# bernborgess/raft-tla

Measured on AMD Instinct MI355X. Metric: distinct states/sec (whole node) + wall time to exhaust, 3-server Raft, higher is better.
Workload: dtype u32

## Files before the change

### raft-tla_amd/csrc/rtla_klevel.h

```cpp
#pragma once
#include "rtla_kdev.h"

namespace {

template <int NS>
__device__ __forceinline__ void add_at(uint32_t* a, uint32_t j, uint32_t v) {
#pragma unroll
  for (int k = 0; k < NS; k++)
    if ((uint32_t)k == j) a[k] += v;
}
template <int NS, int S, class P>
__device__ __forceinline__ int successor_orbit_step_sig(const Layout& L, P prow, const DeltaT<NS>& d,
                                                        const uint32_t* psg, int k, bool all, FP& best) {
  return with_successor<NS>(L, prow, d, [&](auto rec_of, int nmsg, auto slot_of, int nelec, auto elec_of) {
    uint32_t ms[NS], mr[NS];
#pragma unroll
    for (int j = 0; j < NS; j++) {
      ms[j] = psg[(NS + j) * S];
      mr[j] = psg[(2 * NS + j) * S];
    }
#pragma unroll
    for (int q = 0; q < 3; q++) {
      if (q >= d.nops) continue;
      const uint64_t o = d.op_old[q], v = d.op_new[q];
      if (o) {
        const uint32_t c = slot_sig_sent(L, o);
        add_at<NS>(ms, slot_src(L, o), 0u - c);
        add_at<NS>(mr, slot_dst(L, o), 0u - slot_sig_recv(c));
      }
      if (v) {
        const uint32_t c = slot_sig_sent(L, v);
        add_at<NS>(ms, slot_src(L, v), c);
        add_at<NS>(mr, slot_dst(L, v), slot_sig_recv(c));
      }
    }
    const uint32_t lsrv = d.srv >= 0 ? srv_sig<NS>(d.srv, d.rec) : 0u;
    uint64_t sig[NS];
#pragma unroll
    for (int i = 0; i < NS; i++) sig[i] = sig_of(i == d.srv ? lsrv : psg[i * S], ms[i], mr[i]);
    const SymRank r = sym_rank_from<NS>(L, sig, rec_of, nmsg, slot_of, nelec, elec_of);
    const int k1 = all ? r.ncomb : min(k + 1, r.ncomb);
    for (int j = k; j < k1; j++) {
      const FP f = sym_image_fp<NS>(L, rec_of, nmsg, slot_of, nelec, elec_of, r, j);
      if (fp_less(f, best)) best = f;
    }
    return k1 < r.ncomb ? k1 : -1;
  });
}

}

namespace {

constexpr int RING = 128;
constexpr int NEWCAP = 512;
constexpr int NEWFLUSH = NEWCAP - 3 * 64;


__host__ __device__ constexpr int compact_lds_words(int W, int AW, int GROUP, bool sym, bool multi) {
  return (4 * GROUP * (sym ? 2 : 1) + (multi ? 4 * SHARD_MAX : 0) + NEWCAP / 2 + GROUP * W + GROUP * AW +
          RING / 2 * (sym ? 2 : 1) + (sym ? 5 * 64 + 3 * NMAX * GROUP : 0) + 3) & ~3;
}

__device__ __forceinline__ unsigned long long win_bits(unsigned long long bits, int off) {
  if (off >= 64 || off <= -64) return 0ull;
  return off >= 0 ? bits << off : bits >> (-off);
}

template <int NS>
__device__ __forceinline__ unsigned long long cand_mask(const Layout& L, const uint32_t* row, int nmsg, int wb,
                                                        bool dup = true) {
  constexpr int N = NS;
  unsigned long long rv = 0, bl = 0, ldr = 0, tmo = 0;
#pragma unroll
  for (int i = 0; i < N; i++) {
    const uint32_t w0 = srv_w0(L, row, i);
    const uint32_t role = s_role(w0);
    if (role == FOLLOWER || role == CANDIDATE) tmo |= 1ull << i;
    if (role == CANDIDATE) {
      rv |= (unsigned long long)(~s_vresp(w0) & ((1u << N) - 1u)) << (i * N);
      if (__builtin_popcount(s_vgrant(w0)) * 2 > N) bl |= 1ull << i;
    }
    if (role == LEADER) ldr |= 1ull << i;
  }
  unsigned long long ae = 0, cr = 0;
#pragma unroll
  for (int i = 0; i < N; i++)
    if (ldr >> i & 1ull) {
      ae |= (((1ull << N) - 1ull) & ~(1ull << i)) << (i * N);
      cr |= ((1ull << L.V) - 1ull) << (i * L.V);
    }
  const unsigned long long bag = nmsg >= 64 ? ~0ull : ((1ull << nmsg) - 1ull);
  unsigned long long m = 0;
  m |= win_bits((1ull << N) - 1ull, L.fam[F_RESTART] - wb);
  m |= win_bits(tmo, L.fam[F_TIMEOUT] - wb);
  m |= win_bits(rv, L.fam[F_REQUESTVOTE] - wb);
  m |= win_bits(bl, L.fam[F_BECOMELEADER] - wb);
  m |= win_bits(cr, L.fam[F_CLIENTREQUEST] - wb);
  m |= win_bits(ldr, L.fam[F_ADVANCECOMMIT] - wb);
  m |= win_bits(ae, L.fam[F_APPENDENTRIES] - wb);
  m |= win_bits(bag, L.fam[F_RECEIVE] - wb);
  if (dup) m |= win_bits(bag, L.fam[F_DUPLICATE] - wb);
  m |= win_bits(bag, L.fam[F_DROP] - wb);
  return m;
}

__device__ __forceinline__ void outbox_holes(const ShardBox& box, int o, unsigned long long from,
                                             unsigned long long to, int lane) {
  to = min(to, box.cap);
  for (unsigned long long j = from + lane; j < to; j += 64) {
    const unsigned long long k = (unsigned long long)o * box.cap + j;
    box.send_fp[2 * k] = 0ull;
    box.send_fp[2 * k + 1] = 0ull;
  }
}

__device__ __forceinline__ unsigned long long home_slot(const FP& key, int lg) {
  return lg ? key.a >> (64 - lg) : 0ull;
}

}

#ifndef RTLA_COMPACT_WAVES_PER_EU
#define RTLA_COMPACT_WAVES_PER_EU 3
#endif
#ifndef RTLA_SYM_WAVES_PER_EU
#define RTLA_SYM_WAVES_PER_EU 4
#endif

namespace {
struct KeyStep {
  FP f;
  int next;
};
template <int NS, Layout LC, int S>
__device__ __noinline__ KeyStep key_one(const Layout& Lrt, const uint32_t* prow, const uint32_t* psg, int inst, int k,
                                        bool all, FP best0, FP afp) {
  const Layout& L = pick_layout<LC>(Lrt);
  DeltaT<NS> d;
  d.enabled = 0;
  compute_delta<NS>(L, prow, inst, d);
  KeyStep r{FP{0, 0}, -1};
  if (!d.enabled) {
    r.next = -2;
    return r;
  }
  FP best = best0;
  r.next = successor_orbit_step_sig<NS, S>(L, prow, d, psg, k, all, best);
  r.f = r.next < 0 ? fp_add(orbit_key_finish(best), afp) : best;
  return r;
}

struct BuildOut {
  int bad, sub, in_model;
};
template <int NS, Layout LC, int GROUP>
__device__ __noinline__ BuildOut build_one(const Layout& Lrt, const uint32_t* prow, int inst, FP qfp,
                                           const uint32_t* pall_p, uint32_t* d1, uint32_t* base2, int n1, int off,
                                           bool write, bool wait) {
  const Layout& L = pick_layout<LC>(Lrt);
  DeltaT<NS> d;
  d.enabled = 0;
  compute_delta<NS>(L, prow, inst, d);
  const FP cfp = fp_add(qfp, delta_fp<NS>(L, prow, d));
  BuildOut o{check_invariants_v<NS>(L, prow, d.srv, d.rec[0], d.rec[1], d.elec, d.erec[0]), d.sub, d.in_model};
  uint32_t spk[PACKW], epk[PACKW];
  child_pack(L, d, spk, epk);
  if (wait) asm volatile("s_waitcnt vmcnt(0)" ::: "memory");
  if (write)
    child_write(L, prow, d, spk, epk, StridedWords<GROUP>{const_cast<uint32_t*>(pall_p)}, cfp, [&](int w, uint32_t v) {
      const int i = off + w;
      if (i < n1) d1[i] = v;
      else base2[i - n1] = v;
    });
  return o;
}

}

#ifdef RTLA_STAMPS
#define RTLA_STAMP_DECL                                                   \
  unsigned long long st_prev_ = __builtin_amdgcn_s_memtime();              \
  unsigned long long st_acc_[8] = {0, 0, 0, 0, 0, 0, 0, 0};
#define STAMP(k)                                                             \
  do {                                                                       \
    const unsigned long long t_ = __builtin_amdgcn_s_memtime();              \
    st_acc_[k] += t_ - st_prev_;                                             \
    st_prev_ = t_;                                                           \
  } while (0)
#define RTLA_STAMP_FLUSH(ctr, lane)                                          \
  if ((lane) == 0)                                                           \
    for (int k_ = 0; k_ < 8; k_++) atomicAdd(&(ctr)->stamp[k_], st_acc_[k_]);
#else
#define RTLA_STAMP_DECL
#define STAMP(k)
#define RTLA_STAMP_FLUSH(ctr, lane)
#endif

#ifndef RTLA_NARROW_W
#define RTLA_NARROW_W 32
#endif
#ifndef RTLA_NARROW_WAVES
#define RTLA_NARROW_WAVES 4
#endif
constexpr int compact_waves(const Layout& L, bool sym) {
  return sym ? RTLA_SYM_WAVES_PER_EU
             : (L.N != 0 && L.W <= RTLA_NARROW_W ? RTLA_NARROW_WAVES : RTLA_COMPACT_WAVES_PER_EU);
}
template <int NS, bool MULTI, int GROUP, Layout LC, bool SYM>
__global__ void __launch_bounds__(256)
__attribute__((amdgpu_waves_per_eu(compact_waves(LC, SYM))))
k_expand_compact(Layout Lrt, Ring cur, unsigned long long s_begin, unsigned long long s_end,
                 unsigned long long cur_base, Ring next, unsigned long long* __restrict__ parents,
                 unsigned long long next_base, unsigned long long next_cap, unsigned long long* table,
                 unsigned long long* sent, int tlog2, DevCounters* ctr, ShardBox box, int xflags) {
  const Layout& L = pick_layout<LC>(Lrt);
  const int me = box.me;
  extern __shared__ __attribute__((aligned(16))) uint32_t lds[];
  __shared__ unsigned int cov[2 * COVER_CODES];
  const int wave = threadIdx.x >> 6, lane = threadIdx.x & 63;
  const int W = L.W, AW = L.all_words;
  uint32_t* wl = lds + wave * compact_lds_words(W, AW, GROUP, SYM, MULTI);
  FP* pfpl = reinterpret_cast<FP*>(wl);
  FP* afpl = pfpl + GROUP;
  unsigned long long* obox =
      reinterpret_cast<unsigned long long*>(wl + 4 * GROUP * (SYM ? 2 : 1));
  uint16_t* newl = reinterpret_cast<uint16_t*>(obox + (MULTI ? 2 * SHARD_MAX : 0));
  uint32_t* rows = reinterpret_cast<uint32_t*>(newl + NEWCAP);
  uint32_t* pall = rows + GROUP * W;
  const StridedWords<GROUP> pall_mine{pall + (lane & (GROUP - 1))};
  uint16_t* ring = reinterpret_cast<uint16_t*>(pall + GROUP * AW);
  uint16_t* kring = ring + RING;
  int kpos = 0, kdone = 0;
  FP* cbest = reinterpret_cast<FP*>(kring + (SYM ? RING : 0));
  uint32_t* cent = reinterpret_cast<uint32_t*>(cbest + (SYM ? 64 : 0));
  int ccount = 0;
  uint32_t* sigl = cent + (SYM ? 64 : 0);
  if (MULTI) {
    if (lane < SHARD_MAX) {
      obox[lane] = ~0ull;
      obox[SHARD_MAX + lane] = OBOX_CHUNK;
    }
    wave_sync();
  }
  cover_zero(cov, 2 * COVER_CODES);

  unsigned my_gen = 0, my_probe = 0;
  unsigned my_dup = 0;
#ifdef RTLA_COUNT_CAS
  unsigned my_cas = 0;
#endif
  const int ninst = L.fam[F_COUNT];
  const unsigned long long lanes_below = (1ull << lane) - 1ull;
  constexpr bool narrow = !SYM && LC.N != 0 && LC.W <= RTLA_NARROW_W;
  constexpr bool dup_narrow = false;
  const bool dup_counted = (!narrow || dup_narrow) && L.C == 1 && !(xflags & (XF_ALL_SUCCESSORS | XF_NO_CHUNKS));
  const bool recv_group = SYM || L.C > 1;
  constexpr int family_cut = narrow ? 22 : SYM ? 40 : 64;
  RTLA_STAMP_DECL
  bool pend = false;
  unsigned long long pold = 0;
  FP pf{0, 0};
  uint32_t pinfo = 0;
  const bool async_cas = !(xflags & XF_CAS_ONLY);
  bool cpend = false;
  bool cflight = false;
  unsigned long long cold = 0, ckey = 0, cidx = 0;
  uint32_t cinfo = 0;
  int head = 0, tail = 0;
  unsigned long long dedup_new = 0;
  unsigned long long s0 = 0;

  auto chunk_delta = [&](bool active, const uint32_t* prow, int inst, auto& d) {
    const int f0 = inst_family(L, __builtin_amdgcn_readfirstlane(inst));
    const bool one_family = __ballot(active && inst_family(L, inst) != f0) == 0ull;
    if (!one_family || (xflags & XF_GENERIC_DELTA)) {
      if (active) compute_delta<NS>(L, prow, inst, d);
    } else if (active) {
      switch (f0) {
        case F_RESTART: compute_delta<NS, F_RESTART>(L, prow, inst, d); break;
        case F_TIMEOUT: compute_delta<NS, F_TIMEOUT>(L, prow, inst, d); break;
        case F_REQUESTVOTE: compute_delta<NS, F_REQUESTVOTE>(L, prow, inst, d); break;
        case F_BECOMELEADER: compute_delta<NS, F_BECOMELEADER>(L, prow, inst, d); break;
        case F_CLIENTREQUEST: compute_delta<NS, F_CLIENTREQUEST>(L, prow, inst, d); break;
        case F_ADVANCECOMMIT: compute_delta<NS, F_ADVANCECOMMIT>(L, prow, inst, d); break;
        case F_APPENDENTRIES: compute_delta<NS, F_APPENDENTRIES>(L, prow, inst, d); break;
        case F_RECEIVE: compute_delta<NS, F_RECEIVE>(L, prow, inst, d); break;
        case F_DUPLICATE: compute_delta<NS, F_DUPLICATE>(L, prow, inst, d); break;
        default: compute_delta<NS, F_DROP>(L, prow, inst, d); break;
      }
    }
  };
  auto cover_add = [&](unsigned* base, bool on, int inst, int sub) {
    if (xflags & XF_NO_COVER) return;
    const int code = on ? cover_code(L, inst, sub) : -1;
    const unsigned long long m = __ballot(on);
    if (m) {
      const int c0 = __shfl(code, __builtin_ctzll(m));
      const bool same = on && code == c0;
      const int n0 = __popcll(__ballot(same));
      if (lane == 0) atomicAdd(&base[c0], (unsigned)n0);
      if (on && !same) atomicAdd(&base[code], 1u);
    }
  };
  auto build_all = [&]() {
    const int ntot = tail - head;
    if (ntot == 0) return;
    unsigned long long obase = 0;
    if (lane == 0) obase = atomicAdd(&ctr->next_count, (unsigned long long)ntot);
    obase = shfl0_u64(obase);
    if (obase + ntot > next_cap && lane == 0) set_flag(ctr, FLAG_FRONTIER_FULL);
    const int nrows = obase >= next_cap ? 0 : (int)min<unsigned long long>((unsigned long long)ntot, next_cap - obase);
    const bool rows_on = !(xflags & XF_NO_MATERIALIZE) && RTLA_IDX_OK(ctr, obase + nrows, ctr->cap_next + 1);
    const unsigned long long p0 = ring_idx(next, obase);
    const int n1 = (int)min<unsigned long long>(next.cap - p0, (unsigned long long)nrows) * W;
    uint32_t* d1 = next.base + p0 * (unsigned long long)W;
    auto copy_rows = [&](int rb, int re) {
      const int nwords = re * W;
      int r = rb, w = lane;
      while (w >= W) { w -= W; r++; }
      for (int i0 = rb * W; i0 < nwords; i0 += 64) {
        const int i = i0 + lane;
        if (i < nwords) {
          const int sr = newl[(head + r) & (NEWCAP - 1)] >> 8;
          const uint32_t v = rows[sr * W + w];
          if (i < n1) d1[i] = v;
          else next.base[i - n1] = v;
        }
        w += 64;
        while (w >= W) { w -= W; r++; }
      }
    };
    if (rows_on) copy_rows(0, nrows);
    for (int b = 0; b < ntot; b += 64) {
      const bool act = b + lane < ntot;
      const int e = act ? newl[(head + b + lane) & (NEWCAP - 1)] : 0;
      const int sl = e >> 8, inst = e & 255;
      const int child = b + lane;
      if constexpr (SYM) {
        BuildOut o{0, 0, 0};
        if (act)
          o = build_one<NS, LC, GROUP>(Lrt, rows + sl * W, inst, pfpl[sl], pall + sl, d1, next.base, n1, child * W,
                                      rows_on && child < nrows, rows_on && b == 0);
        else if (rows_on && b == 0)
          asm volatile("s_waitcnt vmcnt(0)" ::: "memory");
        if (!(xflags & XF_ALL_SUCCESSORS) && claim_violation(ctr, o.bad, lane))
          record_violation(ctr, cur_base + s0 + sl, inst, 1, child < nrows ? next_base + obase + child : ~0ull);
        cover_add(cov + COVER_CODES, act, inst, o.sub);
        if (child < nrows && RTLA_IDX_OK(ctr, next_base + obase + child, ctr->cap_parents))
          parents[next_base + obase + child] =
              (xflags & XF_ALL_SUCCESSORS)
                  ? (cur_base + s0 + sl) << 32 | (unsigned long long)(o.in_model ? 1u : 0u) << 31 |
                        (unsigned long long)o.sub << 16 | (unsigned long long)inst
                  : (unsigned long long)me << 56 | (cur_base + s0 + sl) << 16 | (unsigned long long)inst;
        continue;
      }
      DeltaT<NS> d;
      d.enabled = 0;
      if (act) compute_delta<NS>(L, rows + sl * W, inst, d);
      const FP qfp = pfpl[sl];
      FP cfp{0, 0};
      int bad = 0;
      if (act) {
        const uint32_t* prow = rows + sl * W;
        cfp = fp_add(qfp, delta_fp<NS>(L, prow, d));
        bad = check_invariants_v<NS>(L, prow, d.srv, d.rec[0], d.rec[1], d.elec, d.erec[0]);
      }
      if (!(xflags & XF_ALL_SUCCESSORS) && claim_violation(ctr, bad, lane))
        record_violation(ctr, cur_base + s0 + sl, inst, 1, child < nrows ? next_base + obase + child : ~0ull);
      cover_add(cov + COVER_CODES, act, inst, d.sub);
      uint32_t spk[PACKW], epk[PACKW];
      if (act) child_pack(L, d, spk, epk);
      if (rows_on) {
        if (b == 0) asm volatile("s_waitcnt vmcnt(0)" ::: "memory");
        if (child < nrows) {
          const StridedWords<GROUP> pall_p{pall + sl};
          const int off = child * W;
          child_write(L, rows + sl * W, d, spk, epk, pall_p, cfp, [&](int w, uint32_t v) {
            const int i = off + w;
            if (i < n1) d1[i] = v;
            else next.base[i - n1] = v;
          });
        }
      }
      if (child < nrows && RTLA_IDX_OK(ctr, next_base + obase + child, ctr->cap_parents))
        parents[next_base + obase + child] =
            (xflags & XF_ALL_SUCCESSORS)
                ? (cur_base + s0 + sl) << 32 | (unsigned long long)(d.in_model ? 1u : 0u) << 31 |
                      (unsigned long long)d.sub << 16 | (unsigned long long)inst
                : (unsigned long long)me << 56 | (cur_base + s0 + sl) << 16 | (unsigned long long)inst;
    }
    head = tail;
  };
  auto issue_cas = [&]() {
#ifdef RTLA_COUNT_CAS
    if (cpend) my_cas++;
#endif
    if (cpend) cold = atomicCAS(&table[cidx], 0ull, ckey);
    cflight = cpend;
    cpend = false;
  };
  auto resolve = [&]() {
    bool isnew = false;
    uint32_t ninfo = pinfo;
    const int powner = MULTI ? fp_owner(pf, box.nshard) : me;
    bool rem = false;
    if (xflags & XF_ALL_SUCCESSORS) {
      isnew = pend;
    } else if (async_cas) {
      if (cflight) {
        if (cold == 0ull) isnew = true;
        else if (cold != ckey)
          isnew = fpset_resolve(table, tlog2, ckey, cidx, cold, ctr);
      }
      ninfo = cinfo;
      cflight = false;
      if (pend) {
        const unsigned long long key = pf.b | 1ull;
        if (MULTI && powner != me) {
          if (pold != key) {
            rem = true;
            if (box.slog2) sent[home_slot(pf, box.slog2)] = key;
          }
        } else if (pold != key) {
          const unsigned long long idx = pf.a >> (64 - tlog2);
          cidx = pold == 0ull ? idx : ((idx + 1ull) & ((1ull << tlog2) - 1ull));
          ckey = key;
          cinfo = pinfo;
          cpend = true;
        }
      }
    } else if (pend) {
      if (MULTI && powner != me) {
        rem = pold != (pf.b | 1ull);
        if (rem && box.slog2) sent[home_slot(pf, box.slog2)] = pf.b | 1ull;
      } else {
        const unsigned long long pidx = pf.a >> (64 - tlog2);
        isnew = (xflags & XF_CAS_ONLY) ? fpset_resolve(table, tlog2, pf.b | 1ull, pidx, pold, ctr)
                                       : fpset_resolve_loaded(table, tlog2, pf.b | 1ull, pidx, pold, ctr);
      }
    }
    if (MULTI) {
      const uint32_t rinfo = pinfo;
      if (__ballot(rem)) {
        unsigned long long mym = 0;
        int ocnt = 0;
        for (int o = 0; o < box.nshard; o++) {
          const unsigned long long m = __ballot(rem && powner == o);
          if (powner == o) mym = m;
          if (lane == o) ocnt = __popcll(m);
        }
        unsigned long long b1 = 0, b2 = 0;
        int room = 0;
        if (ocnt > 0) {
          const unsigned long long b = obox[lane], used = obox[SHARD_MAX + lane];
          room = b == ~0ull ? 0 : (int)(OBOX_CHUNK - used);
          b1 = b + used;
          if (ocnt > room) {
            b2 = atomicAdd(&box.out_count[lane], (unsigned long long)OBOX_CHUNK);
            obox[lane] = b2;
            obox[SHARD_MAX + lane] = (unsigned long long)(ocnt - room);
          } else {
            obox[SHARD_MAX + lane] = used + (unsigned long long)ocnt;
          }
        }
        const int src = rem ? powner : 0;
        b1 = shfl_u64(b1, src);
        b2 = shfl_u64(b2, src);
        room = __shfl(room, src);
        const int r = __popcll(mym & lanes_below);
        const unsigned long long slot = r < room ? b1 + r : b2 + (r - room);
        const unsigned long long ref = outbox_ref(s0 + (rinfo >> 16), rinfo & 0xffffu);
        if (rem && slot < box.cap) outbox_put(box, powner, slot, pf, ref);
        const bool ov = rem && slot >= box.cap;
        const unsigned long long om = __ballot(ov);
        if (om) {
          unsigned long long ob = 0;
          if (lane == 0) ob = atomicAdd(box.over_count, (unsigned long long)__popcll(om));
          ob = shfl0_u64(ob);
          if (ov) {
            const unsigned long long k = ob + __popcll(om & lanes_below);
            if (k < box.over_cap) {
              box.over_fp[2 * k] = pf.a;
              box.over_fp[2 * k + 1] = pf.b;
              box.over_ref[k] = ref;
            } else {
              set_flag(ctr, FLAG_OUTBOX_FULL);
            }
          }
        }
      }
    }
    const unsigned long long m = __ballot(isnew);
    if (m && (xflags & XF_DEDUP_ONLY)) {
      dedup_new += __popcll(m);
    } else if (m) {
      if (isnew) newl[(tail + __popcll(m & lanes_below)) & (NEWCAP - 1)] = (uint16_t)((ninfo >> 16) << 8 | (ninfo & 255u));
      tail += __popcll(m);
      wave_sync();
    }
    pend = false;
  };

  bool nprobe = false;
  unsigned long long nidx = 0;
  FP ncf{0, 0};
  int nowner = me;
  uint32_t ninfo_new = 0;
  auto eval_chunk = [&](int done, int cnt) {
    const bool active = lane < cnt;
    const int e = active ? ring[(done + lane) & (RING - 1)] : 0;
    const int sl = e >> 8, inst = e & 255;
    const uint32_t* prow = rows + sl * W;
    const FP qfp = pfpl[sl];
    DeltaFpT<NS> d;
    d.enabled = 0;
    if (!(xflags & XF_NO_DELTA)) chunk_delta(active, prow, inst, d);
    const bool en = enabled_ok(&ctr->flags, d.enabled != 0, d.err);
    my_gen += en ? 1u : 0u;
    bool kq = false;
    nprobe = false;
    nidx = 0;
    ncf = FP{0, 0};
    nowner = me;
    ninfo_new = (uint32_t)sl << 16 | (uint32_t)inst;
    if (en && (xflags & XF_ALL_SUCCESSORS)) {
      nprobe = true;
    } else if (en && d.in_model) {
      const FP cfp = (xflags & XF_NO_HASH) ? FP{qfp.a + d.rec[0] + (uint64_t)d.fmsg.a, qfp.b + d.rec[1]}
                                           : fp_add(qfp, delta_fp<NS>(L, prow, d));
      const FP qfp0 = row_fp(prow);
      if (cfp.a != qfp0.a || cfp.b != qfp0.b) {
        if constexpr (SYM) {
          kq = true;
        } else {
          const FP key = cfp;
          nprobe = !(xflags & XF_NO_PROBE);
          ncf = key;
          nowner = MULTI ? fp_owner(key, box.nshard) : me;
          nidx = (MULTI && nowner != me) ? home_slot(key, box.slog2) : key.a >> (64 - tlog2);
        }
      }
    }
    if constexpr (SYM) {
      const unsigned long long km = __ballot(kq);
      if (kq) kring[(kpos + __popcll(km & lanes_below)) & (RING - 1)] = (uint16_t)(sl << 8 | inst);
      kpos += __popcll(km);
    }
    cover_add(cov, en, inst, d.sub);
    int bad = 0;
    if (en && !d.in_model && !(xflags & (XF_DEDUP_ONLY | XF_ALL_SUCCESSORS)))
      bad = check_invariants_v<NS>(L, prow, d.srv, d.rec[0], d.rec[1], d.elec, d.erec[0]);
    if (claim_violation(ctr, bad, lane)) record_violation(ctr, cur_base + s0 + sl, inst, 0, ~0ull);
  };
  auto key_chunk = [&](int kd, int kc, bool last) {
    const int cn = ccount;
    const bool cont = lane < cn;
    const bool active = lane < cn + kc;
    int e = 0, k = 0;
    if (cont) {
      const uint32_t ce = cent[lane];
      e = (int)(ce & 0xffffu);
      k = (int)(ce >> 16);
    } else if (active) {
      e = kring[(kd + lane - cn) & (RING - 1)];
    }
    const int sl = e >> 8, inst = e & 255;
    const uint32_t* prow = rows + sl * W;
    nprobe = false;
    ninfo_new = (uint32_t)sl << 16 | (uint32_t)inst;
    int next = -1;
    FP best{~0ull, ~0ull};
    if (active) {
      const KeyStep ks = key_one<NS, LC, GROUP>(Lrt, prow, sigl + sl, inst, k, last,
                                                cont ? cbest[lane] : FP{~0ull, ~0ull}, afpl[sl]);
      next = ks.next < 0 ? -1 : ks.next;
      best = ks.f;
      if (ks.next == -1) {
        const FP key = ks.f;
        nprobe = !(xflags & XF_NO_PROBE);
        ncf = key;
        nowner = MULTI ? fp_owner(key, box.nshard) : me;
        nidx = (MULTI && nowner != me) ? home_slot(key, box.slog2) : key.a >> (64 - tlog2);
      }
    }
    const unsigned long long cm = __ballot(next >= 0);
    wave_sync();
    if (next >= 0) {
      const int c = __popcll(cm & lanes_below);
      cent[c] = (uint32_t)e | (uint32_t)next << 16;
      cbest[c] = best;
    }
    ccount = __popcll(cm);
    wave_sync();
  };
  auto issue_probe = [&]() {
    asm volatile("" ::: "memory");
    issue_cas();
    if (nprobe) {
      my_probe++;
      pend = true;
      pf = ncf;
      pinfo = ninfo_new;
      unsigned long long* slotp = &((MULTI && nowner != me) ? sent : table)[nidx];
      if (MULTI && nowner != me && !box.slog2)
        pold = 0ull;
      else if (!(xflags & XF_ALL_SUCCESSORS))
        pold = ((xflags & XF_CAS_ONLY) && !(MULTI && nowner != me))
                   ? atomicCAS(slotp, 0ull, ncf.b | 1ull)
                   : __hip_atomic_load(slotp, __ATOMIC_RELAXED, __HIP_MEMORY_SCOPE_AGENT);
    }
    nprobe = false;
  };
  auto drain = [&]() {
    resolve();
    if (async_cas) {
      issue_cas();
      resolve();
    }
  };
  auto append_instance = [&](int& pos, unsigned long long mask, int wb, int q, const uint32_t* prow_mine, int f) {
    const bool mine = (mask >> q) & 1ull;
    if (recv_group && f == F_RECEIVE) {
      const uint32_t ty = mine ? slot_type(L, prow_mine, wb + q - L.fam[F_RECEIVE]) : 0u;
#pragma unroll
      for (uint32_t t = 0; t < 4; t++) {
        const bool b = mine && ty == t;
        const unsigned long long m = __ballot(b);
        if (b) ring[(pos + __popcll(m & lanes_below)) & (RING - 1)] = (uint16_t)(lane << 8 | (wb + q));
        pos += __popcll(m);
      }
    } else {
      const unsigned long long m = __ballot(mine);
      if (mine) ring[(pos + __popcll(m & lanes_below)) & (RING - 1)] = (uint16_t)(lane << 8 | (wb + q));
      pos += __popcll(m);
    }
  };

  auto take_group = [&]() -> unsigned long long {
    const bool full = MULTI && lane < box.nshard && lane != me &&
                      __hip_atomic_load(&box.out_count[lane], __ATOMIC_RELAXED, __HIP_MEMORY_SCOPE_AGENT) >= box.stop_at;
    unsigned long long g = ~0ull;
    if (!__ballot(full) && lane == 0) g = atomicAdd(&ctr->group_next, 1ull);
    return g;
  };
  if (MULTI && blockIdx.x == 0 && lane == 0 && wave == 0) ctr->group_size = GROUP;
  unsigned long long gnext = 0;
  if (MULTI) gnext = take_group();
  else if (lane == 0) gnext = atomicAdd(&ctr->group_next, 1ull);
  const unsigned long long ngroups = (s_end - s_begin + GROUP - 1) / GROUP;
  for (unsigned long long gi = shfl0_u64(gnext); gi < ngroups; gi = shfl0_u64(gnext)) {
    if (!MULTI && lane == 0) gnext = atomicAdd(&ctr->group_next, 1ull);
    s0 = s_begin + gi * GROUP;
    const int nvalid = (int)min<unsigned long long>((unsigned long long)GROUP, s_end - s0);
    {
      const uint32_t* src = ring_row(cur, s0, W);
      const int nw = nvalid * W;
      if (RTLA_IDX_OK(ctr, ring_idx(cur, s0) + nvalid, cur.cap + 1)) copy_words_lds16(rows, src, nw, lane);
    }
    wave_sync();
    unsigned long long gnn = MULTI ? 0ull : shfl0_u64(gnext);
    const bool valid = lane < nvalid;
    const uint32_t* prow_mine = rows + (lane & (GROUP - 1)) * W;
    int nmsg = 0;
    if (valid) {
      pfpl[lane] = fp_add(row_fp(prow_mine), alllogs_delta<NS>(L, prow_mine, pall_mine));
      if (SYM) afpl[lane] = alllogs_fp(L, pall_mine);
      nmsg = row_nmsg(L, prow_mine);
      if constexpr (SYM) {
        uint32_t loc[NS], ms[NS], mr[NS];
        sym_sig_parts<NS>(L, [&](int i, uint32_t* out) { load_rec<NS>(L, prow_mine, i, out); }, nmsg,
                          [&](int q) { return slot_raw(L, prow_mine, q); }, loc, ms, mr);
#pragma unroll
        for (int j = 0; j < NS; j++) {
          sigl[j * GROUP + lane] = loc[j];
          sigl[(NS + j) * GROUP + lane] = ms[j];
          sigl[(2 * NS + j) * GROUP + lane] = mr[j];
        }
      }
    }
    wave_sync();
    STAMP(0);
    if (dup_counted) {
      if constexpr (SYM) {
        if (valid) my_gen += (unsigned)nmsg;
        if (!(xflags & XF_NO_COVER)) {
          int nd = valid ? nmsg : 0;
          for (int off = 32; off > 0; off >>= 1) nd += __shfl_down(nd, off);
          if (lane == 0 && nd) atomicAdd(&cov[F_DUPLICATE], (unsigned)nd);
        }
      } else if (valid) {
        my_dup += (unsigned)nmsg;
      }
    }
    for (int wb = 0; wb < ((xflags & XF_NO_CHUNKS) ? 0 : ninst); wb += 64) {
      const unsigned long long mask = valid ? cand_mask<NS>(L, prow_mine, nmsg, wb, !dup_counted) : 0ull;
      unsigned long long todo = wave_or_u64(mask);
      int pos = 0, done = 0;
      while (todo || pos > done) {
        int cfam = -1;
        while (todo && pos - done < 64) {
          const int q = __builtin_ctzll(todo);
          const int f = inst_family(L, wb + q);
          if (f != cfam && pos - done >= family_cut) break;
          cfam = f;
          todo &= todo - 1;
          append_instance(pos, mask, wb, q, prow_mine, f);
        }
        const int cnt = min(64, pos - done);
        wave_sync();
        STAMP(1);
        eval_chunk(done, cnt);
        STAMP(2);
        if (!SYM || (xflags & XF_ALL_SUCCESSORS)) {
          resolve();
          STAMP(3);
          issue_probe();
          STAMP(4);
        } else {
          while (kpos - kdone + ccount >= 64) {
            const int kc = min(kpos - kdone, 64 - ccount);
            key_chunk(kdone, kc, kc == 0);
            kdone += kc;
            STAMP(7);
            resolve();
            STAMP(3);
            issue_probe();
            STAMP(4);
          }
        }
        if (tail - head > NEWFLUSH) {
          drain();
          build_all();
          STAMP(5);
        }
        done += cnt;
      }
    }
    uint32_t pfa = 0, pfb = 0;
    if (MULTI) {
      gnext = take_group();
      gnn = shfl0_u64(gnext);
    }
    while (SYM && kpos - kdone + ccount > 0) {
      const int kc = min(kpos - kdone, 64 - ccount);
      key_chunk(kdone, kc, kc == 0 || kpos - kdone + ccount <= 64);
      kdone += kc;
      STAMP(7);
      resolve();
      issue_probe();
    }
    if (gnn < ngroups) {
      const unsigned long long sn = s_begin + gnn * GROUP;
      const int lines = ((int)min<unsigned long long>((unsigned long long)GROUP, s_end - sn) * W + 31) / 32;
      const uint32_t* pa = ring_row(cur, sn, W) + 32 * min(lane, lines - 1);
      const uint32_t* pb = ring_row(cur, sn, W) + 32 * min(lane + 64, lines - 1);
      pfa = __hip_atomic_load(pa, __ATOMIC_RELAXED, __HIP_MEMORY_SCOPE_AGENT);
      pfb = __hip_atomic_load(pb, __ATOMIC_RELAXED, __HIP_MEMORY_SCOPE_AGENT);
    }
    drain();
    if constexpr (!SYM) STAMP(7);
    build_all();
    asm volatile("s_waitcnt vmcnt(0)" ::: "memory");
    asm volatile("" ::"v"(pfa), "v"(pfb));
    wave_sync();
    STAMP(6);
  }
  if (MULTI) {
    for (int o = 0; o < box.nshard; o++) {
      const unsigned long long b = obox[o], used = obox[SHARD_MAX + o];
      if (b != ~0ull) outbox_holes(box, o, b + used, b + OBOX_CHUNK, lane);
    }
  }
  for (int off = 32; off > 0; off >>= 1) {
    my_gen += __shfl_down(my_gen, off);
    my_probe += __shfl_down(my_probe, off);
    my_dup += __shfl_down(my_dup, off);
  }
  my_gen += my_dup;
  if (lane == 0 && my_dup && !(xflags & XF_NO_COVER)) atomicAdd(&cov[F_DUPLICATE], my_dup);
  if (lane == 0 && my_gen) atomicAdd(&ctr->generated, (unsigned long long)my_gen);
  if (lane == 0 && my_probe) atomicAdd(&ctr->probes, (unsigned long long)my_probe);
  if (lane == 0 && dedup_new) atomicAdd(&ctr->next_count, dedup_new);
#ifdef RTLA_COUNT_CAS
  for (int off = 32; off > 0; off >>= 1) my_cas += __shfl_down(my_cas, off);
  if (lane == 0 && my_cas) atomicAdd(&ctr->cas, (unsigned long long)my_cas);
#endif
  STAMP(7);
  RTLA_STAMP_FLUSH(ctr, lane)
  cover_flush(cov, 2 * COVER_CODES, ctr->cover);
}

namespace rtla {

#ifndef RTLA_GROUP64_LDS
#define RTLA_GROUP64_LDS (16 * 1024)
#endif
constexpr int compact_group(const Layout& L) {
  if (L.sym) return 32;
  return compact_lds_words(L.W, L.all_words, 64, false, true) * sizeof(uint32_t) <= RTLA_GROUP64_LDS ? 64 : 32;
}
#ifndef RTLA_GROUP32_LDS
#define RTLA_GROUP32_LDS (19 * 1024)
#endif
#ifndef RTLA_SYM_GROUP
#define RTLA_SYM_GROUP 16
#endif
constexpr int spec_group(const Layout& L) {
  if (L.sym) return RTLA_SYM_GROUP;
  const int g = compact_group(L);
  return g == 32 && compact_lds_words(L.W, L.all_words, 32, L.sym, true) * sizeof(uint32_t) > RTLA_GROUP32_LDS ? 16 : g;
}

template <int NS, int GROUP, Layout LC, bool SYM = false>
static hipError_t launch_compact(const LevelArgs& a) {
  const Layout& L = a.L;
  const bool multi = a.box.nshard > 1;
  const int xflags = a.xflags;
  const int wpb = (xflags & XF_BLOCK4) ? expand_compact_wpb(L) : 1;
  const uint64_t s_begin = a.s_begin, s_end = a.s_end;
  DevCounters* ctr = a.ctr;
  hipStream_t st = a.st;
  auto kfn = multi ? k_expand_compact<NS, true, GROUP, LC, SYM> : k_expand_compact<NS, false, GROUP, LC, SYM>;
  const uint64_t groups = (s_end - s_begin + GROUP - 1) / GROUP;
  uint64_t blocks = std::min<uint64_t>((groups + wpb - 1) / wpb, 1u << 20);
  const size_t lds = (size_t)wpb * compact_lds_words(L.W, L.all_words, GROUP, SYM, multi) * sizeof(uint32_t);
  if (!(xflags & XF_NO_PERSIST) || a.query) {
    static int per_cu[2][2];
    int& pc = per_cu[multi][wpb == 1];
    if (!pc) {
      if (hipOccupancyMaxActiveBlocksPerMultiprocessor(&pc, kfn, 64 * wpb, lds) != hipSuccess || pc < 1)
        pc = 16 / wpb;
      if (const char* e = getenv("RTLA_BLOCKS_PER_CU"))
        if (atoi(e) > 0) pc = std::min(pc, atoi(e));
    }
    blocks = std::min<uint64_t>(blocks, (uint64_t)device_cus() * pc);
    if (a.query) {
      a.query[0] = device_cus() * pc * wpb;
      a.query[1] = GROUP;
      return hipSuccess;
    }
  }
  {
    hipError_t e = hipMemsetAsync(&ctr->group_next, 0, sizeof(ctr->group_next), st);
    if (e != hipSuccess) return e;
  }
  hipLaunchKernelGGL(kfn, dim3((unsigned)blocks), dim3(64 * wpb), lds, st, L, a.cur, (unsigned long long)s_begin,
                     (unsigned long long)s_end, (unsigned long long)a.cur_base, a.out.next,
                     (unsigned long long*)a.out.parents, (unsigned long long)a.out.next_base,
                     (unsigned long long)a.out.next_cap, (unsigned long long*)a.table, (unsigned long long*)a.sent, a.tlog2, ctr, a.box, xflags);
  return hipGetLastError();
}

}
```

Measured before the change: 3.068 billion.

## Write non-narrow child rows directly with vector stores, skip parent copy and prefetch wait

For non-narrow layouts, each child row is now assembled word by word and written with 16-byte packed stores straight into the output ring. Previously the parent rows were bulk-copied into the output and then patched by scattered writes. The next-group prefetch loads are no longer waited on at the end of the group; their consumption is deferred to after the next group's LDS copy, so they overlap the build. Duplicate counting is also enabled for narrow layouts. The per-word select logic adds ALU work, and the deferred prefetch changes how register lifetimes and waitcnt interact.

```diff
diff --git a/raft-tla_amd/csrc/rtla_klevel.h b/raft-tla_amd/csrc/rtla_klevel.h
--- a/raft-tla_amd/csrc/rtla_klevel.h
+++ b/raft-tla_amd/csrc/rtla_klevel.h
@@ -151,13 +151,67 @@
   return r;
 }
 
+__device__ __forceinline__ uint32_t pack_word(const uint32_t* a, int k) {
+  uint32_t v = a[0];
+#pragma unroll
+  for (int j = 1; j < PACKW; j++)
+    if (k == j) v = a[j];
+  return v;
+}
+template <class P, class R, int NR>
+__device__ __forceinline__ uint32_t child_word(const Layout& L, P prow, const DeltaT<NR>& d, const uint32_t* spk,
+                                               const uint32_t* epk, R all_new, FP fp, int ne, int w) {
+  if (w < 4)
+    return w == 0 ? (uint32_t)fp.a : w == 1 ? (uint32_t)(fp.a >> 32) : w == 2 ? (uint32_t)fp.b : (uint32_t)(fp.b >> 32);
+  if (w == L.off_hdr) return (uint32_t)d.nmsg | (uint32_t)ne << 8;
+  if (w >= L.off_all && w < L.off_elec) return all_new[w - L.off_all];
+  uint32_t v = prow[w];
+  if (w < L.off_all) {
+    const int i = (w - L.off_srv) / L.srv_w;
+    if (d.srv == i) v = pack_word(spk, w - L.off_srv - i * L.srv_w);
+  } else if (w < L.off_bag) {
+    const int e = (w - L.off_elec) / L.elec_w;
+    if (d.elec && e == ne - 1) v = pack_word(epk, w - L.off_elec - e * L.elec_w);
+  } else {
+    const int q = (w - L.off_bag) / L.slot_w;
+    const bool hi = w - L.off_bag - q * L.slot_w != 0;
+#pragma unroll
+    for (int o = 0; o < 3; o++)
+      if (o < d.nops && d.op_slot[o] == q) v = hi ? (uint32_t)(d.op_new[o] >> 32) : (uint32_t)d.op_new[o];
+  }
+  return v;
+}
+struct __attribute__((packed, aligned(4))) RowWords4 {
+  uint32_t v[4];
+};
+template <bool FIXED, class P, class R, int NR>
+__device__ __forceinline__ void child_store(const Layout& L, P prow, const DeltaT<NR>& d, const uint32_t* spk,
+                                            const uint32_t* epk, R all_new, FP fp, uint32_t* dst) {
+  const int ne = row_nelec(L, prow) + (d.elec ? 1 : 0);
+  auto store4 = [&](int w) {
+    RowWords4 t;
+#pragma unroll
+    for (int k = 0; k < 4; k++) t.v[k] = child_word(L, prow, d, spk, epk, all_new, fp, ne, w + k);
+    *reinterpret_cast<RowWords4*>(dst + w) = t;
+  };
+  int w = 0;
+  if constexpr (FIXED) {
+#pragma unroll
+    for (; w + 4 <= L.W; w += 4) store4(w);
+#pragma unroll
+    for (; w < L.W; w++) dst[w] = child_word(L, prow, d, spk, epk, all_new, fp, ne, w);
+  } else {
+    for (; w + 4 <= L.W; w += 4) store4(w);
+    for (; w < L.W; w++) dst[w] = child_word(L, prow, d, spk, epk, all_new, fp, ne, w);
+  }
+}
+
 struct BuildOut {
   int bad, sub, in_model;
 };
 template <int NS, Layout LC, int GROUP>
 __device__ __noinline__ BuildOut build_one(const Layout& Lrt, const uint32_t* prow, int inst, FP qfp,
-                                           const uint32_t* pall_p, uint32_t* d1, uint32_t* base2, int n1, int off,
-                                           bool write, bool wait) {
+                                           const uint32_t* pall_p, uint32_t* dst) {
   const Layout& L = pick_layout<LC>(Lrt);
   DeltaT<NS> d;
   d.enabled = 0;
@@ -166,13 +220,7 @@
   BuildOut o{check_invariants_v<NS>(L, prow, d.srv, d.rec[0], d.rec[1], d.elec, d.erec[0]), d.sub, d.in_model};
   uint32_t spk[PACKW], epk[PACKW];
   child_pack(L, d, spk, epk);
-  if (wait) asm volatile("s_waitcnt vmcnt(0)" ::: "memory");
-  if (write)
-    child_write(L, prow, d, spk, epk, StridedWords<GROUP>{const_cast<uint32_t*>(pall_p)}, cfp, [&](int w, uint32_t v) {
-      const int i = off + w;
-      if (i < n1) d1[i] = v;
-      else base2[i - n1] = v;
-    });
+  if (dst) child_store<LC.N != 0>(L, prow, d, spk, epk, StridedWords<GROUP>{const_cast<uint32_t*>(pall_p)}, cfp, dst);
   return o;
 }
 
@@ -253,8 +301,7 @@
   const int ninst = L.fam[F_COUNT];
   const unsigned long long lanes_below = (1ull << lane) - 1ull;
   constexpr bool narrow = !SYM && LC.N != 0 && LC.W <= RTLA_NARROW_W;
-  constexpr bool dup_narrow = false;
-  const bool dup_counted = (!narrow || dup_narrow) && L.C == 1 && !(xflags & (XF_ALL_SUCCESSORS | XF_NO_CHUNKS));
+  const bool dup_counted = L.C == 1 && !(xflags & (XF_ALL_SUCCESSORS | XF_NO_CHUNKS));
   const bool recv_group = SYM || L.C > 1;
   constexpr int family_cut = narrow ? 22 : SYM ? 40 : 64;
   RTLA_STAMP_DECL
@@ -315,6 +362,7 @@
     const unsigned long long p0 = ring_idx(next, obase);
     const int n1 = (int)min<unsigned long long>(next.cap - p0, (unsigned long long)nrows) * W;
     uint32_t* d1 = next.base + p0 * (unsigned long long)W;
+    auto row_at = [&](int c) { return c * W < n1 ? d1 + c * W : next.base + (c * W - n1); };
     auto copy_rows = [&](int rb, int re) {
       const int nwords = re * W;
       int r = rb, w = lane;
@@ -331,7 +379,8 @@
         while (w >= W) { w -= W; r++; }
       }
     };
-    if (rows_on) copy_rows(0, nrows);
+    if constexpr (narrow)
+      if (rows_on) copy_rows(0, nrows);
     for (int b = 0; b < ntot; b += 64) {
       const bool act = b + lane < ntot;
       const int e = act ? newl[(head + b + lane) & (NEWCAP - 1)] : 0;
@@ -340,10 +389,8 @@
       if constexpr (SYM) {
         BuildOut o{0, 0, 0};
         if (act)
-          o = build_one<NS, LC, GROUP>(Lrt, rows + sl * W, inst, pfpl[sl], pall + sl, d1, next.base, n1, child * W,
-                                      rows_on && child < nrows, rows_on && b == 0);
-        else if (rows_on && b == 0)
-          asm volatile("s_waitcnt vmcnt(0)" ::: "memory");
+          o = build_one<NS, LC, GROUP>(Lrt, rows + sl * W, inst, pfpl[sl], pall + sl,
+                                      rows_on && child < nrows ? row_at(child) : nullptr);
         if (!(xflags & XF_ALL_SUCCESSORS) && claim_violation(ctr, o.bad, lane))
           record_violation(ctr, cur_base + s0 + sl, inst, 1, child < nrows ? next_base + obase + child : ~0ull);
         cover_add(cov + COVER_CODES, act, inst, o.sub);
@@ -371,18 +418,21 @@
       cover_add(cov + COVER_CODES, act, inst, d.sub);
       uint32_t spk[PACKW], epk[PACKW];
       if (act) child_pack(L, d, spk, epk);
-      if (rows_on) {
-        if (b == 0) asm volatile("s_waitcnt vmcnt(0)" ::: "memory");
-        if (child < nrows) {
-          const StridedWords<GROUP> pall_p{pall + sl};
-          const int off = child * W;
-          child_write(L, rows + sl * W, d, spk, epk, pall_p, cfp, [&](int w, uint32_t v) {
-            const int i = off + w;
-            if (i < n1) d1[i] = v;
-            else next.base[i - n1] = v;
-          });
-        }
-      }
+      if constexpr (narrow) {
+        if (rows_on) {
+          if (b == 0) asm volatile("s_waitcnt vmcnt(0)" ::: "memory");
+          if (child < nrows) {
+            const StridedWords<GROUP> pall_p{pall + sl};
+            const int off = child * W;
+            child_write(L, rows + sl * W, d, spk, epk, pall_p, cfp, [&](int w, uint32_t v) {
+              const int i = off + w;
+              if (i < n1) d1[i] = v;
+              else next.base[i - n1] = v;
+            });
+          }
+        }
+      } else if (rows_on && child < nrows)
+        child_store<LC.N != 0>(L, rows + sl * W, d, spk, epk, StridedWords<GROUP>{pall + sl}, cfp, row_at(child));
       if (child < nrows && RTLA_IDX_OK(ctr, next_base + obase + child, ctr->cap_parents))
         parents[next_base + obase + child] =
             (xflags & XF_ALL_SUCCESSORS)
@@ -649,6 +699,7 @@
   if (MULTI) gnext = take_group();
   else if (lane == 0) gnext = atomicAdd(&ctr->group_next, 1ull);
   const unsigned long long ngroups = (s_end - s_begin + GROUP - 1) / GROUP;
+  [[maybe_unused]] uint32_t pfa_c = 0, pfb_c = 0;
   for (unsigned long long gi = shfl0_u64(gnext); gi < ngroups; gi = shfl0_u64(gnext)) {
     if (!MULTI && lane == 0) gnext = atomicAdd(&ctr->group_next, 1ull);
     s0 = s_begin + gi * GROUP;
@@ -658,6 +709,8 @@
       const int nw = nvalid * W;
       if (RTLA_IDX_OK(ctr, ring_idx(cur, s0) + nvalid, cur.cap + 1)) copy_words_lds16(rows, src, nw, lane);
     }
+    if constexpr (!narrow)
+      asm volatile("" ::"v"(pfa_c), "v"(pfb_c));
     wave_sync();
     unsigned long long gnn = MULTI ? 0ull : shfl0_u64(gnext);
     const bool valid = lane < nvalid;
@@ -737,7 +790,8 @@
         done += cnt;
       }
     }
-    uint32_t pfa = 0, pfb = 0;
+    [[maybe_unused]] uint32_t pfa = 0, pfb = 0;
+    pfa_c = pfb_c = 0;
     if (MULTI) {
       gnext = take_group();
       gnn = shfl0_u64(gnext);
@@ -755,14 +809,21 @@
       const int lines = ((int)min<unsigned long long>((unsigned long long)GROUP, s_end - sn) * W + 31) / 32;
       const uint32_t* pa = ring_row(cur, sn, W) + 32 * min(lane, lines - 1);
       const uint32_t* pb = ring_row(cur, sn, W) + 32 * min(lane + 64, lines - 1);
-      pfa = __hip_atomic_load(pa, __ATOMIC_RELAXED, __HIP_MEMORY_SCOPE_AGENT);
-      pfb = __hip_atomic_load(pb, __ATOMIC_RELAXED, __HIP_MEMORY_SCOPE_AGENT);
+      if constexpr (narrow) {
+        pfa = __hip_atomic_load(pa, __ATOMIC_RELAXED, __HIP_MEMORY_SCOPE_AGENT);
+        pfb = __hip_atomic_load(pb, __ATOMIC_RELAXED, __HIP_MEMORY_SCOPE_AGENT);
+      } else {
+        pfa_c = __hip_atomic_load(pa, __ATOMIC_RELAXED, __HIP_MEMORY_SCOPE_AGENT);
+        pfb_c = __hip_atomic_load(pb, __ATOMIC_RELAXED, __HIP_MEMORY_SCOPE_AGENT);
+      }
     }
     drain();
     if constexpr (!SYM) STAMP(7);
     build_all();
-    asm volatile("s_waitcnt vmcnt(0)" ::: "memory");
-    asm volatile("" ::"v"(pfa), "v"(pfb));
+    if constexpr (narrow) {
+      asm volatile("s_waitcnt vmcnt(0)" ::: "memory");
+      asm volatile("" ::"v"(pfa), "v"(pfb));
+    }
     wave_sync();
     STAMP(6);
   }
```

New measurement: 3.453 billion (median of 6 runs). +12.5%, better.
